# MycroftAI/mycroft-precise

Measured on AMD Instinct MI355X. Metric: MFCC+GRU windows/sec (node); max concurrent real-time 16 kHz streams, higher is better.
Workload: dtype f32

## Files before the change

include/precise_engine.h:

```cpp
#ifndef PRECISE_ENGINE_H
#define PRECISE_ENGINE_H

#include <stddef.h>
#include <stdint.h>

#ifdef __cplusplus
extern "C" {
#endif

#define PE_ABI_VERSION 8

typedef enum pe_status {
    PE_OK = 0,
    PE_ERR_INVALID = 1,
    PE_ERR_HIP = 2,
    PE_ERR_UNSUPPORTED = 3,
    PE_ERR_NOMEM = 4,
    PE_ERR_EOF = 5
} pe_status;

typedef struct pe_params {
    int32_t sample_rate;
    int32_t window_samples;
    int32_t hop_samples;
// ... 133 lines not shown
int pe_set_trigger_model(pe_engine* e, int32_t model, int32_t chunk_size_bytes, double sensitivity, int32_t trigger_level);
int pe_decode_device(pe_engine* e, const float* raw_dev, double* conf_out_dev, unsigned char* fired_out_dev, void* hip_stream);
int pe_decode(pe_engine* e, const float* raw_host, double* conf_out_host, unsigned char* fired_out_host);

typedef struct pe_info {
    int32_t n_streams, n_features, n_mfcc, units, n_layers, ring_slots, carry_capacity;
    int32_t mfcc_precision, gru_precision;
    int64_t device_bytes;
} pe_info;
int pe_get_info(const pe_engine* e, pe_info* out);

int pe_get_stream_state(pe_engine* e, int32_t* q_out, uint32_t* computed_out, uint32_t* emitted_out);

int pe_set_renumber_at(pe_engine* e, uint32_t call_number);

int pe_set_fused(pe_engine* e, int32_t enabled);

int pe_set_input_projection(pe_engine* e, int32_t enabled);

int pe_set_gru_waves(pe_engine* e, int32_t waves_per_tile);

int pe_set_gru_tiling(pe_engine* e, int32_t tiling);
int pe_get_gru_tiling(const pe_engine* e);

int pe_set_timing(pe_engine* e, int32_t enabled);
int pe_get_last_timing(pe_engine* e, float* mfcc_ms, float* gru_ms);

#define PE_TRAIN_MAX_MODELS 16
typedef struct pe_trainer pe_trainer;
int pe_trainer_create(int32_t n_features, int32_t feature_size, const pe_weights* init, int32_t device, pe_trainer** out);
int pe_trainer_create_models(int32_t n_features, int32_t feature_size, const pe_weights* init, int32_t n_models, int32_t device,
                             pe_trainer** out);
int pe_trainer_create_wide(int32_t n_features, int32_t feature_size, const pe_weights* init, int32_t n_models, int32_t device,
                           pe_trainer** out);
int pe_trainer_destroy(pe_trainer* t);
const char* pe_trainer_last_error(const pe_trainer* t);
int pe_trainer_n_models(const pe_trainer* t);
int pe_trainer_n_params(const pe_trainer* t);
int pe_trainer_n_params_model(const pe_trainer* t, int32_t m);

int pe_trainer_get_weights(pe_trainer* t, float* flat_out);
int pe_trainer_set_weights(pe_trainer* t, const float* flat);
int pe_trainer_get_accumulators(pe_trainer* t, float* flat_out);
int pe_trainer_reset_optimizer(pe_trainer* t);

int pe_trainer_loss_grad(pe_trainer* t, const float* feats_host, const float* targets_host, int32_t n, const float* masks_host,
// ... 124 lines not shown
```

mycroft_precise_amd/_lib.py:

```python
import ctypes as C
import importlib.util
import os
import weakref

import numpy as np

HERE = os.path.dirname(os.path.abspath(__file__))
LIB_PATH = os.environ.get('PE_LIB') or os.path.join(HERE, 'libprecise_engine.so')

PE_OK, PE_ERR_INVALID, PE_ERR_HIP, PE_ERR_UNSUPPORTED, PE_ERR_NOMEM, PE_ERR_EOF = range(6)
ABI_VERSION = 8


class PeParams(C.Structure):
    _fields_ = [(n, C.c_int32) for n in (
        'sample_rate', 'window_samples', 'hop_samples', 'n_fft', 'n_filt', 'n_mfcc', 'n_features',
        'use_delta', 'mfcc_precision', 'gru_precision', 'vectorizer', 'ring_precision')]


class PeGruLayer(C.Structure):
    _fields_ = [('n_in', C.c_int32), ('units', C.c_int32),
                ('kernel', C.POINTER(C.c_float)), ('recurrent_kernel', C.POINTER(C.c_float)),
                ('bias', C.POINTER(C.c_float))]

# ... 71 lines not shown
    'pe_evaluate_clips': (C.c_int, [C.c_void_p, C.c_void_p, C.c_int32, C.c_void_p, C.c_int32, C.c_int32, C.c_void_p, C.c_int64]),
    'pe_simulate_scores': (C.c_int, [C.c_void_p, C.c_void_p, C.c_int64, C.c_void_p, C.c_int32, C.c_double, C.c_double, C.c_int32,
                                     C.c_int32, C.c_void_p, C.c_int32, C.c_void_p, C.c_void_p]),
    'pe_simulate_clips': (C.c_int, [C.c_void_p, C.c_void_p, C.c_int32, C.c_void_p, C.c_int32, C.c_int32, C.c_double, C.c_double,
                                    C.c_int32, C.c_int32, C.c_void_p, C.c_int32, C.c_void_p, C.c_void_p, C.c_void_p, C.c_int64]),
    'pe_stats_scores': (C.c_int, [C.c_void_p, C.c_void_p, C.c_int32, C.c_int64, C.c_void_p, C.c_int64, C.c_void_p, C.c_int32, C.c_int32,
                                  C.c_void_p, C.c_void_p]),
    'pe_test_clips': (C.c_int, [C.c_void_p, C.c_void_p, C.c_int32, C.c_void_p, C.c_int32, C.c_int64, C.c_void_p, C.c_void_p, C.c_int32,
                                C.c_int32, C.c_void_p, C.c_void_p, C.c_void_p]),
    'pe_set_decoder': (C.c_int, [C.c_void_p, C.c_void_p, C.c_int32, C.c_int32, C.c_int32, C.c_double]),
    'pe_set_trigger': (C.c_int, [C.c_void_p, C.c_int32, C.c_double, C.c_int32]),
    'pe_set_decoder_model': (C.c_int, [C.c_void_p, C.c_int32, C.c_void_p, C.c_int32, C.c_int32, C.c_int32, C.c_double]),
    'pe_set_trigger_model': (C.c_int, [C.c_void_p, C.c_int32, C.c_int32, C.c_double, C.c_int32]),
    'pe_decode_device': (C.c_int, [C.c_void_p, C.c_void_p, C.c_void_p, C.c_void_p, C.c_void_p]),
    'pe_decode': (C.c_int, [C.c_void_p, C.c_void_p, C.c_void_p, C.c_void_p]),
    'pe_get_info': (C.c_int, [C.c_void_p, C.POINTER(PeInfo)]),
    'pe_get_stream_state': (C.c_int, [C.c_void_p, C.c_void_p, C.c_void_p, C.c_void_p]),
    'pe_set_fused': (C.c_int, [C.c_void_p, C.c_int32]),
    'pe_set_gru_waves': (C.c_int, [C.c_void_p, C.c_int32]),
    'pe_set_gru_tiling': (C.c_int, [C.c_void_p, C.c_int32]),
    'pe_get_gru_tiling': (C.c_int, [C.c_void_p]),
    'pe_set_input_projection': (C.c_int, [C.c_void_p, C.c_int32]),
    'pe_set_timing': (C.c_int, [C.c_void_p, C.c_int32]),
    'pe_get_last_timing': (C.c_int, [C.c_void_p, C.POINTER(C.c_float), C.POINTER(C.c_float)]),
    'pe_trainer_create': (C.c_int, [C.c_int32, C.c_int32, C.POINTER(PeWeights), C.c_int32, C.POINTER(C.c_void_p)]),
    'pe_trainer_destroy': (C.c_int, [C.c_void_p]),
    'pe_trainer_last_error': (C.c_char_p, [C.c_void_p]),
    'pe_trainer_n_params': (C.c_int, [C.c_void_p]),
    'pe_trainer_get_weights': (C.c_int, [C.c_void_p, C.c_void_p]),
    'pe_trainer_set_weights': (C.c_int, [C.c_void_p, C.c_void_p]),
    'pe_trainer_get_accumulators': (C.c_int, [C.c_void_p, C.c_void_p]),
    'pe_trainer_reset_optimizer': (C.c_int, [C.c_void_p]),
    'pe_trainer_loss_grad': (C.c_int, [C.c_void_p, C.c_void_p, C.c_void_p, C.c_int32, C.c_void_p, C.c_float, C.c_void_p, C.c_void_p,
                                       C.c_void_p]),
    'pe_trainer_apply': (C.c_int, [C.c_void_p, C.c_void_p, C.c_float, C.c_float, C.c_float, C.c_int32]),
    'pe_trainer_set_data': (C.c_int, [C.c_void_p, C.c_void_p, C.c_void_p, C.c_int32]),
    'pe_trainer_step': (C.c_int, [C.c_void_p, C.c_void_p, C.c_int32, C.c_float, C.c_uint64, C.c_uint64, C.c_float, C.c_float,
                                  C.c_float, C.c_float, C.c_int32, C.c_void_p]),
    'pe_trainer_evaluate': (C.c_int, [C.c_void_p, C.c_void_p, C.c_void_p, C.c_int32, C.c_float, C.c_void_p, C.c_void_p, C.c_void_p]),
    'pe_trainer_create_models': (C.c_int, [C.c_int32, C.c_int32, C.POINTER(PeWeights), C.c_int32, C.c_int32, C.POINTER(C.c_void_p)]),
    'pe_trainer_create_wide': (C.c_int, [C.c_int32, C.c_int32, C.POINTER(PeWeights), C.c_int32, C.c_int32, C.POINTER(C.c_void_p)]),
    'pe_trainer_n_models': (C.c_int, [C.c_void_p]),
    'pe_trainer_n_params_model': (C.c_int, [C.c_void_p, C.c_int32]),
    'pe_trainer_step_models': (C.c_int, [C.c_void_p, C.c_void_p, C.c_int32, C.c_uint64, C.POINTER(PeTrainHparams), C.c_void_p]),
    'pe_trainer_n_samples': (C.c_int, [C.c_void_p, C.c_int32]),
    'pe_trainer_set_validation': (C.c_int, [C.c_void_p, C.c_void_p, C.c_void_p, C.c_int32]),
# ... 549 lines not shown

    def stream_state(self):
        q = np.empty(self.n_streams, dtype=np.int32)
        kc = np.empty(self.n_streams, dtype=np.uint32)
        ke = np.empty(self.n_streams, dtype=np.uint32)
        self._check(self._lib.pe_get_stream_state(self._h, q.ctypes.data, kc.ctypes.data, ke.ctypes.data))
        return q, kc, ke

    def set_fused(self, enabled: bool):
        self._check(self._lib.pe_set_fused(self._h, int(bool(enabled))))

    def set_input_projection(self, enabled: bool):
        self._check(self._lib.pe_set_input_projection(self._h, int(bool(enabled))))

    def set_gru_waves(self, waves: int):
        self._check(self._lib.pe_set_gru_waves(self._h, int(waves)))

    def set_gru_tiling(self, tiling: int):
        self._check(self._lib.pe_set_gru_tiling(self._h, int(tiling)))

    def gru_tiling(self) -> int:
        return int(self._lib.pe_get_gru_tiling(self._h))

    def set_timing(self, enabled: bool):
        self._check(self._lib.pe_set_timing(self._h, int(bool(enabled))))

    def last_timing(self):
        a, b = C.c_float(0), C.c_float(0)
        self._check(self._lib.pe_get_last_timing(self._h, C.byref(a), C.byref(b)))
        return a.value, b.value

    def close(self):
        if getattr(self, '_h', None) and self._h.value:
            if getattr(self, '_views', 0) > 0:
                self._close_pending = True
                try:
                    self._lib.pe_wait(self._h)
                except Exception:
                    pass
                return
            for miner in list(getattr(self, '_miners', ())):
                miner.close()
            self._lib.pe_destroy(self._h)
            self._h = C.c_void_p()

    def __del__(self):
# ... 530 lines not shown
```

mycroft_precise_amd/csrc/engine.hip:

```cpp
#include "../../include/precise_engine.h"
#include "pe_common.h"
#include "gru_cw_pack.h"
#include "mfcc_general_device.h"
#include "gru_train_device.h"
#include "gru_train_wide_device.h"
#include "mine_device.h"
#include "sample_device.h"
#include "generate_device.h"
#include "augment_device.h"
#include "stats_device.h"

#include <algorithm>
#include <cmath>
#include <cstdarg>
#include <cstdio>
#include <cstdlib>
#include <cstring>
#include <string>
#include <vector>

using namespace pe;

namespace {

// ... 23 lines not shown
    double threshold = 0.5; int level = 3, rearm = -8; bool on = false;
};

}

struct pe_engine {
    pe_params prm{};
    int device = 0;
    int n_streams = 0, n_tiles = 0, n_padded = 0;
    int units = 0, n_in = 0, n_layers = 0;
    int ring_slots = 0;
    int mel_nnz = 0;
    std::string err;
    std::vector<void*> allocs;
    std::vector<size_t> alloc_bytes;
    int64_t device_bytes = 0;
    StreamRec* rec = nullptr;
    int16_t* carry = nullptr;
    const int16_t* kept = nullptr; int kept_chunk = 0;
    const int16_t* call_head = nullptr; int call_head_chunk = 0; bool call_keep = false;
    uint32_t call_no = 1;
    uint32_t renumber_at = 0x7fff0000u;
    bool fused = true;
    int gru_waves = 0;
    bool general = false;
    int row_floats = kRowFloats;
    int carry_cap = kCarryCap;
    GeneralTables gtab{};
    int gru_tiling = -1;
    int n_cus = 256;
    float* ring = nullptr;
    float* proj_ring = nullptr;
    bool proj_ok = false, proj_on = false;
    std::vector<float> proj_w_host, proj_b_host;
    int max_updates = 1;
    uint32_t* ke_hist = nullptr;
    unsigned char* table_blob = nullptr;
    pe_wave::Layout table_layout{};
    int n_models = 1;
    std::vector<NetPack> nets;
    std::vector<DecState> dec;
    bool wide = false;
    int wide_kx4[2] = {1, 1};
    int layer_units[2] = {0, 0}, layer_n_in[2] = {0, 0}, wide_units = 0;
    std::vector<double> mel_host;
    int32_t* activation = nullptr;
// ... 609 lines not shown
    WaveTables<R> t;
    t.blob = e->table_blob;
    t.L = e->table_layout;
    return t;
}

int max_frames_per_call(const pe_engine* e, long long new_samples) {
    const long long fmax = ((long long)(e->carry_cap - 1) + new_samples - frame_len_of(e->prm)) / e->prm.hop_samples + 1;
    return (int)(fmax < 1 ? 1 : fmax);
}

StreamState state_of(const pe_engine* e, uint32_t call) {
    StreamState st;
    st.rec = e->rec; st.carry = e->carry; st.n_padded = (uint32_t)e->n_padded; st.call = call;
    return st;
}

int begin_state_call(pe_engine* e, hipStream_t s, uint32_t* call) {
    if (e->call_no >= e->renumber_at) {
        PE_HIP(e, launch_renumber(state_of(e, e->call_no + 1u), e->n_padded, s));
        e->call_no = 2u;
    }
    *call = ++e->call_no;
    return PE_OK;
}

template <class R>
MfccStreamArgs<R> mfcc_args(const pe_engine* e, const int16_t* pcm_dev, int chunk, uint32_t call, const int32_t* ids = nullptr, int n_active = 0) {
    MfccStreamArgs<R> a;
    a.geo = geom(e);
    if (ids) a.geo.n_streams = n_active;
    a.pcm = pcm_dev;
    a.chunk = chunk;
    a.pcm_pairs_ok = ((chunk & 1) == 0) && ((reinterpret_cast<uintptr_t>(pcm_dev) & 3u) == 0);
    a.ids = ids;
    a.st = state_of(e, call);
    a.head = ids ? nullptr : e->call_head; a.head_chunk = e->call_head_chunk; a.keep = (!ids && e->call_keep) ? 1 : 0;
    a.ring = e->ring; a.ring_bf16 = e->prm.ring_precision;
    a.proj_ring = e->proj_on ? e->proj_ring : nullptr;
    a.n_updates = 1; a.ke_hist = nullptr; a.n_padded = e->n_padded;
    a.n_frame_rows = max_frames_per_call(e, chunk);
    a.div_hop = FastDiv::make((uint32_t)e->prm.hop_samples);
    a.div_chunk = FastDiv::make((uint32_t)chunk);
    return a;
}

// ... 195 lines not shown
int flush_kept(pe_engine* e, hipStream_t s) {
    if (!e->kept) return PE_OK;
    PE_HIP(e, launch_materialize_carry(state_of(e, e->call_no + 1u), e->kept, e->kept_chunk, e->n_streams, s));
    e->kept = nullptr; e->kept_chunk = 0;
    return PE_OK;
}

bool keep_eligible(const pe_engine* e, const int16_t* pcm_dev, int chunk) {
    return !e->general && (chunk & 1) == 0 && (reinterpret_cast<uintptr_t>(pcm_dev) & 3u) == 0 && chunk >= frame_len_of(e->prm) - 1
        && chunk >= e->carry_cap - 1;
}

bool can_fuse(const pe_engine* e, int chunk) {
    if (!(e->fused && !e->general && !e->wide && e->table_layout.mel_pad == 10 && chunk <= emit_window(e->prm) - frame_len_of(e->prm))) return false;
    if (gru_args(e).x3) return false;
    if (e->prm.gru_precision == 0 && gru_small_regs(e->units) >= 6 && gru_args(e).waves_per_tile != 4) return false;
    if (e->prm.use_delta && e->prm.gru_precision == 0) {
        const GruArgs g = gru_args(e);
        if (g.cw && (g.waves_per_tile != 4 || e->ring_slots != kCwSlots || e->prm.n_features > kCwSlots)) return false;
    }
    return true;
}

int do_update(pe_engine* e, const int16_t* pcm_dev, int chunk, float* raw_out_dev, float* feats_out_dev,
              hipStream_t s, const int32_t* ids = nullptr, int n_active = 0, bool keep = false) {
    int rc;
    const bool t = e->timing;
    const bool keep_call = keep && !ids && keep_eligible(e, pcm_dev, chunk);
    if (keep_call && e->kept) {
        const char* a0 = reinterpret_cast<const char*>(e->kept);
        const char* a1 = a0 + (size_t)e->n_streams * e->kept_chunk * sizeof(int16_t);
        const char* b0 = reinterpret_cast<const char*>(pcm_dev);
        const char* b1 = b0 + (size_t)e->n_streams * chunk * sizeof(int16_t);
        if (b0 < a1 && a0 < b1)
            return fail(e, PE_ERR_INVALID, "pe_update_device_keep: this call's chunks overlap the previous call's (%p), which still hold the "
                        "streams' leftover samples -- alternate between at least two buffers, or use pe_update_device", (const void*)e->kept);
    }
    if (!keep_call && (rc = flush_kept(e, s))) return rc;
    e->call_head = keep_call ? e->kept : nullptr; e->call_head_chunk = e->kept_chunk; e->call_keep = keep_call;
    struct Reset { pe_engine* e; ~Reset() { e->call_head = nullptr; e->call_head_chunk = 0; e->call_keep = false; } } reset{e};
    e->kept = keep_call ? pcm_dev : nullptr; e->kept_chunk = keep_call ? chunk : 0;
    uint32_t call = 0;
    if ((rc = begin_state_call(e, s, &call))) return rc;
    if (t) { PE_HIP(e, hipEventRecord(e->ev[0], s)); }
    if (raw_out_dev && can_fuse(e, chunk)) {
        GruArgs g = gru_args(e);
        g.call = call;
        g.predict_ke = 1;
        g.chunk = chunk;
        g.out = raw_out_dev;
        if (ids) { g.ids = ids; g.n_streams = n_active; }
        const ModelSet ms = model_set(e, g);
        const ModelSet* const models = e->n_models > 1 ? &ms : nullptr;
        if (e->prm.mfcc_precision == 0) PE_HIP(e, launch_fused(mfcc_args<double>(e, pcm_dev, chunk, call, ids, n_active), tables<double>(e), g, e->n_cus, s, models, e->n_models));
        else PE_HIP(e, launch_fused(mfcc_args<float>(e, pcm_dev, chunk, call, ids, n_active), tables<float>(e), g, e->n_cus, s, models, e->n_models));
        if (t) { PE_HIP(e, hipEventRecord(e->ev[1], s)); PE_HIP(e, hipEventRecord(e->ev[2], s)); e->ev_valid = true; e->ev_has_gru = false; }
    } else {
        if ((rc = launch_mfcc(e, pcm_dev, chunk, s, call, ids, n_active))) return rc;
        if (t) { PE_HIP(e, hipEventRecord(e->ev[1], s)); }
        if (raw_out_dev) {
            if ((rc = launch_gru_ring(e, raw_out_dev, s, ids, n_active))) return rc;
        }
        if (t) { PE_HIP(e, hipEventRecord(e->ev[2], s)); e->ev_valid = true; e->ev_has_gru = raw_out_dev != nullptr; }
    }
    if (feats_out_dev) {
        GatherArgs g{e->n_streams, e->prm.n_features, e->prm.n_mfcc, e->ring_slots, e->prm.ring_precision, e->ring, state_of(e, e->call_no + 1u), feats_out_dev, e->row_floats};
        PE_HIP(e, launch_gather(g, s));
    }
// ... 191 lines not shown
    if (out) *out = nullptr;
    if (n_models < 1 || n_models > kMaxModels) return fail(nullptr, PE_ERR_INVALID, "n_models must be in 1..%d, got %d", kMaxModels, n_models);
    if (!weights) return fail(nullptr, PE_ERR_INVALID, "null argument to pe_create_models");
    return create_engine(p, mel_filters, weights, n_models, n_streams, device, out);
}

int pe_get_n_models(const pe_engine* e) { return e ? e->n_models : -1; }

int pe_set_weights(pe_engine* e, const pe_weights* w, int32_t model) {
    if (!e) return PE_ERR_INVALID;
    if (!w || !w->layers || !w->dense_kernel) return fail(e, PE_ERR_INVALID, "null argument to pe_set_weights");
    if (model < 0 || model >= e->n_models) return fail(e, PE_ERR_INVALID, "model %d outside 0..%d", model, e->n_models - 1);
    if (w->n_layers != e->n_layers) return fail(e, PE_ERR_INVALID, "pe_set_weights: n_layers=%d, the engine's network has %d", w->n_layers, e->n_layers);
    for (int l = 0; l < e->n_layers; ++l) {
        const pe_gru_layer& L = w->layers[l];
        if (!L.kernel || !L.recurrent_kernel || !L.bias) return fail(e, PE_ERR_INVALID, "pe_set_weights: null weight pointer");
        if (L.units != e->layer_units[l] || L.n_in != e->layer_n_in[l])
            return fail(e, PE_ERR_INVALID, "pe_set_weights: layer %d is n_in=%d units=%d, the engine's is n_in=%d units=%d (a live engine takes the widths it was created with)",
                        l, L.n_in, L.units, e->layer_n_in[l], e->layer_units[l]);
    }
    PE_HIP(e, hipSetDevice(e->device));
    PE_DRAIN(e);
    PE_HIP(e, hipDeviceSynchronize());
    int rc = pack_model(e, e->nets[(size_t)model], w, e->wide, e->wide_units);
    if (rc) return rc;
    if (e->proj_ok && model == 0 && !e->general) {
        pack_projection_rows(e, w->layers[0]);
        rc = e->prm.mfcc_precision == 0 ? build_tables<double>(e, e->mel_host.data()) : build_tables<float>(e, e->mel_host.data());
        if (rc) return rc;
        if (e->proj_on)
            PE_HIP(e, launch_project_rows(e->ring, e->proj_ring, reinterpret_cast<const float*>(e->table_blob + e->table_layout.proj_w),
                                          reinterpret_cast<const float*>(e->table_blob + e->table_layout.proj_b), e->prm.n_mfcc,
                                          (long long)e->n_tiles * e->ring_slots * kTileStreams, nullptr));
        PE_HIP(e, hipStreamSynchronize(nullptr));
    }
    return PE_OK;
}

int pe_destroy(pe_engine* e) {
    if (!e) return PE_OK;
    (void)hipSetDevice(e->device);
    (void)drain_async(e);
    for (void* p : e->allocs) (void)hipFree(p);
    for (DeviceBuf* b : {&e->st_pcm, &e->st_out, &e->st_feats, &e->st_mask, &e->st_audio, &e->st_mfcc, &e->st_conf, &e->st_fired, &e->st_ids, &e->st_clips, &e->st_recs, &e->st_pred, &e->st_sim, &e->st_simw, &e->st_stats})
        if (b->p) (void)hipFree(b->p);
    for (auto& ev : e->ev) if (ev) (void)hipEventDestroy(ev);
// ... 1005 lines not shown
    PE_HIP(e, hipDeviceSynchronize());
    const int pending = pending_frames(e->prm);
    const long long frames = ((long long)max_updates * max_chunk_samples + e->prm.hop_samples - 1) / e->prm.hop_samples + 1;
    const int slots = next_pow2((int)(e->prm.n_features + pending + frames));
    if (slots != e->ring_slots) {
        dev_free(e, e->ring, ring_floats(e) * sizeof(float));
        e->ring = nullptr;
        dev_free(e, e->proj_ring, (size_t)e->n_tiles * e->ring_slots * kTileStreams * kProjRow * sizeof(float));
        e->proj_ring = nullptr;
        e->ring_slots = slots;
        int rc = dev_alloc(e, &e->ring, ring_floats(e));
        if (rc) return rc;
        if (e->proj_on && (rc = dev_alloc(e, &e->proj_ring, (size_t)e->n_tiles * e->ring_slots * kTileStreams * kProjRow))) return rc;
    }
    if (!e->ke_hist || max_updates > e->max_updates) {
        if (e->ke_hist) {
            dev_free(e, e->ke_hist, (size_t)e->max_updates * e->n_padded * sizeof(uint32_t));
            e->ke_hist = nullptr;
        }
        int rc = dev_alloc(e, &e->ke_hist, (size_t)max_updates * e->n_padded);
        if (rc) return rc;
    }
    e->max_updates = max_updates;
    return pe_clear(e, nullptr);
}

int pe_update_many_device(pe_engine* e, const int16_t* pcm_dev, int32_t chunk, int32_t n_updates, float* raw_out_dev, void* stream) {
    int rc = check_chunk(e, pcm_dev, chunk);
    if (rc) return rc;
    if (!raw_out_dev || n_updates < 1) return fail(e, PE_ERR_INVALID, "bad arguments to pe_update_many_device");
    if (n_updates > e->max_updates || !e->ke_hist) return fail(e, PE_ERR_INVALID, "call pe_reserve_updates(e, >= %d, >= %d) first", n_updates, chunk);
    PE_HIP(e, hipSetDevice(e->device));
    PE_DRAIN(e);
    const int flen = frame_len_of(e->prm);
    const int pending = pending_frames(e->prm);
    const long long frames = ((long long)n_updates * chunk + e->prm.hop_samples - 1) / e->prm.hop_samples + 1;
    if ((long long)n_updates * chunk >= (1ll << 30)) return fail(e, PE_ERR_INVALID, "n_updates * chunk_samples must stay below 2^30");
    if (e->prm.n_features + pending + frames > e->ring_slots) return fail(e, PE_ERR_INVALID, "reserved ring too small for %d updates of %d samples", n_updates, chunk);
    hipStream_t s = static_cast<hipStream_t>(stream);
    note_user_stream(e, stream);
    if ((rc = flush_kept(e, s))) return rc;
    uint32_t call = 0;
    if ((rc = begin_state_call(e, s, &call))) return rc;
    if (e->general) {
        if (e->prm.mfcc_precision == 0) {
            GeneralStreamArgs<double> a = general_args<double>(e, pcm_dev, chunk, call);
// ... 88 lines not shown
    PE_HIP(e, hipMemcpy(host.data(), e->rec, host.size() * sizeof(StreamRec), hipMemcpyDeviceToHost));
    const uint32_t call = e->call_no + 1u;
    for (int s = 0; s < e->n_streams; ++s) {
        const StreamRec& r0 = host[rec_at((uint32_t)e->n_padded, s, 0)];
        const StreamRec& r1 = host[rec_at((uint32_t)e->n_padded, s, 1)];
        const StreamRec& c = (call - r1.wcall) - 1u < (call - r0.wcall) - 1u ? r1 : r0;
        if (q_out) q_out[s] = c.q;
        if (computed_out) computed_out[s] = c.kc;
        if (emitted_out) emitted_out[s] = c.ke;
    }
    return PE_OK;
}

int pe_set_renumber_at(pe_engine* e, uint32_t call_number) {
    if (!e) return PE_ERR_INVALID;
    if (call_number < 8u || call_number > 0x7fff0000u) return fail(e, PE_ERR_INVALID, "renumbering threshold must be in 8..0x7fff0000");
    e->renumber_at = call_number;
    return PE_OK;
}

int pe_set_fused(pe_engine* e, int32_t enabled) {
    if (!e) return PE_ERR_INVALID;
    PE_DRAIN(e);
    e->fused = enabled != 0;
    return PE_OK;
}

int pe_set_input_projection(pe_engine* e, int32_t enabled) {
    if (!e) return PE_ERR_INVALID;
    if (enabled != 0 && enabled != 1) return fail(e, PE_ERR_INVALID, "input projection must be 0 or 1");
    if (enabled && !e->proj_ok) return fail(e, PE_ERR_UNSUPPORTED, "input-projection rows exist for the float32 network of 17..20 units without delta features only");
    if (enabled && e->n_models > 1) return fail(e, PE_ERR_UNSUPPORTED, "input-projection rows are per model: an engine of %d models has none", e->n_models);
    if ((enabled != 0) == e->proj_on) return PE_OK;
    PE_HIP(e, hipSetDevice(e->device));
    PE_DRAIN(e);
    PE_HIP(e, hipDeviceSynchronize());
    e->proj_on = enabled != 0;
    if (e->proj_on && !e->proj_ring) {
        int rc = dev_alloc(e, &e->proj_ring, (size_t)e->n_tiles * e->ring_slots * kTileStreams * kProjRow);
        if (rc) { e->proj_on = false; return rc; }
    }
    return pe_clear(e, nullptr);
}

int pe_set_gru_waves(pe_engine* e, int32_t waves) {
    if (!e) return PE_ERR_INVALID;
    if (waves != 0 && waves != 1 && waves != 4) return fail(e, PE_ERR_INVALID, "gru kernel shape must be 0 (auto), 1 or 4 (waves per tile)");
    PE_DRAIN(e);
    e->gru_waves = waves;
    return PE_OK;
}

int pe_set_gru_tiling(pe_engine* e, int32_t tiling) {
    if (!e) return PE_ERR_INVALID;
    if (tiling < -1 || tiling > 2) return fail(e, PE_ERR_INVALID, "gru tiling must be -1 (auto), 0 (classic), 1 (re-tiled) or 2 (XDL form)");
    if (e->wide && e->prm.gru_precision == 1) {
        if (tiling != 0) return fail(e, PE_ERR_UNSUPPORTED, "the bf16-operand wide network (gru_precision = 1) has one form, 0; forms 0 (f32-input MFMAs) and 2 (float32 products on the bf16 pipe) belong to the float32 wide network");
        return PE_OK;
    }
    if (e->wide) {
        if (tiling == 1) return fail(e, PE_ERR_UNSUPPORTED, "wide networks have two forms: 0 (f32-input MFMAs) and 2 (float32 products on the bf16 pipe)");
        PE_DRAIN(e);
        e->gru_tiling = tiling;
        return PE_OK;
    }
    if (tiling == 2 && !e->nets[0].x3_blob)
        return fail(e, PE_ERR_UNSUPPORTED, "the XDL form of the float32 network (tiling 2) takes <= 20 units, <= 15 inputs, float32 operands, no use_delta");
    if (tiling == 1 && e->prm.gru_precision == 1 && !e->nets[0].b20_blob)
        return fail(e, PE_ERR_UNSUPPORTED, "the five-values layout of the bf16 network (tiling 1) takes <= 20 units and <= 14 features");
    PE_DRAIN(e);
    e->gru_tiling = tiling;
    return PE_OK;
}

int pe_get_gru_tiling(const pe_engine* e) {
    if (!e) return -2;
    if (e->wide) return e->prm.gru_precision == 0 && wide_uses_x3(e) ? 2 : 0;
    if (e->prm.gru_precision != 0) return gru_args(e).b20 ? 1 : 0;
    const GruArgs a = gru_args(e);
    return a.x3 ? 2 : a.cw ? 1 : 0;
}

int pe_set_timing(pe_engine* e, int32_t enabled) {
    if (!e) return PE_ERR_INVALID;
    e->timing = enabled != 0;
    e->ev_valid = false;
    return PE_OK;
}

int pe_get_last_timing(pe_engine* e, float* mfcc_ms, float* gru_ms) {
    if (!e) return PE_ERR_INVALID;
    if (!e->ev_valid) return fail(e, PE_ERR_INVALID, "no timed update recorded (call pe_set_timing(e, 1) first)");
    PE_HIP(e, hipEventSynchronize(e->ev[2]));
    float a = 0.f, b = 0.f;
    PE_HIP(e, hipEventElapsedTime(&a, e->ev[0], e->ev[1]));
    PE_HIP(e, hipEventElapsedTime(&b, e->ev[1], e->ev[2]));
    if (mfcc_ms) *mfcc_ms = a;
    if (gru_ms) *gru_ms = e->ev_has_gru ? b : 0.f;
    return PE_OK;
}

}

static_assert(PE_TRAIN_MAX_MODELS == kTrainMaxModels, "the header's cap is the kernel table's length");

struct TrainSet {
    const float* feats = nullptr;
    const float* targets = nullptr;
    int n = 0;
// ... 1681 lines not shown
```

mycroft_precise_amd/csrc/kernels.hip:

```cpp
#include <cstdlib>
#include <type_traits>
#include "mfcc_device.h"
#include "mfcc_wave_device.h"
#include "gru_device.h"
#include "gru_cw_device.h"
#include "gru_bf16_device.h"
#include "gru_b20_device.h"
#include "gru_x3_device.h"
#include "gru_wide_device.h"
#include "gru_wide_x3_device.h"
#include "gru_wide_bf16_device.h"
#include "mfcc_general_device.h"
#include "gru_train_device.h"

namespace pe {

#ifndef PE_FRAME_WPE
#define PE_FRAME_WPE 4
#endif
template <int BYTES>
__device__ __forceinline__ void touch_kernel_arguments() {
    const int* ka = (const int*)__builtin_amdgcn_kernarg_segment_ptr();
    static_assert(BYTES <= 12 * 64, "more lines than this helper requests");
    auto line = [&](int i) -> int { return i * 64 < BYTES ? ka[i * 16] : 0; };
    const int v0 = line(0), v1 = line(1), v2 = line(2), v3 = line(3), v4 = line(4), v5 = line(5), v6 = line(6), v7 = line(7),
              v8 = line(8), v9 = line(9), v10 = line(10), v11 = line(11);
    asm volatile("" :: "s"(v0), "s"(v1), "s"(v2), "s"(v3), "s"(v4), "s"(v5), "s"(v6), "s"(v7), "s"(v8), "s"(v9), "s"(v10), "s"(v11));
}
// ... 352 lines not shown
        } else {
            const int tile = bl * 4 + wave;
            if (tile < n_tiles) gru_tile<RG, kRing, PROJ>(gm, tile, threadIdx.x & 63);
        }
    } else if (b < n_net + n_frame_blocks) {
        mfcc_frame_tasks<R, SH, true, !PROJ>(m, t, smem, (b - n_net) * kFrameWaves, n_frame_blocks * kFrameWaves, CW && MW && (frames_first & kBySimd));
    } else {
        mfcc_book_tile<R>(m, b - n_net - n_frame_blocks);
    }
}

#define PE_FUSED_PARAMS (const MfccStreamArgs<R> m, const WaveTables<R> t, const GruArgs g, const int n_gru_blocks, const int n_frame_blocks, const int n_tiles, const int frames_first)
#define PE_FUSED_MODELS_PARAMS (const MfccStreamArgs<R> m, const WaveTables<R> t, const GruArgs g, const int n_gru_blocks, const int n_models, const int n_frame_blocks, \
                                const int n_tiles, const int frames_first, const ModelSet ms)
PE_KERNEL_PAIR((template <class R, class SH, bool DELTA, bool RB>), PE_FRAME_KERNEL(256, PE_FRAME_WPE), fused_update_bf16_kernel, PE_FUSED_PARAMS,
               { fused_update_bf16_body<R, SH, DELTA, RB, false>(m, t, g, nullptr, n_gru_blocks, 1, n_frame_blocks, n_tiles, frames_first); })
PE_KERNEL_PAIR((template <class R, class SH, bool DELTA, bool RB>), PE_FRAME_KERNEL(256, PE_FRAME_WPE), fused_update_bf16_models_kernel, PE_FUSED_MODELS_PARAMS,
               { fused_update_bf16_body<R, SH, DELTA, RB, true>(m, t, g, &ms, n_gru_blocks, n_models, n_frame_blocks, n_tiles, frames_first); })
PE_KERNEL_PAIR((template <class R, class SH, int RG, bool MW, bool PROJ, bool CW = false>), PE_FRAME_KERNEL(256, PE_FRAME_WPE), fused_update_kernel, PE_FUSED_PARAMS,
               { fused_update_body<R, SH, RG, MW, PROJ, CW, false>(m, t, g, nullptr, n_gru_blocks, 1, n_frame_blocks, n_tiles, frames_first); })
PE_KERNEL_PAIR((template <class R, class SH, int RG, bool MW, bool CW>), PE_FRAME_KERNEL(256, PE_FRAME_WPE), fused_update_models_kernel, PE_FUSED_MODELS_PARAMS,
               { fused_update_body<R, SH, RG, MW, false, CW, true>(m, t, g, &ms, n_gru_blocks, n_models, n_frame_blocks, n_tiles, frames_first); })


static int frame_blocks(long long n_tasks, int n_cus, int per_cu = 4) {
    const long long need = (n_tasks + kFrameWaves - 1) / kFrameWaves;
    const long long cap = (long long)n_cus * per_cu;
    return (int)(need < cap ? (need < 1 ? 1 : need) : cap);
}

static int stream_frame_blocks(int n_streams, int n_cus, int per_cu_default = 4) {
    const long long slots = 2LL * n_streams;
    const long long cap_waves = (long long)frame_blocks(slots, n_cus, per_cu_default) * kFrameWaves;
    const long long per_wave = (slots + cap_waves - 1) / cap_waves;
    const long long waves = (slots + per_wave - 1) / per_wave;
    return (int)((waves + kFrameWaves - 1) / kFrameWaves);
}

template <class R>
static size_t frame_lds(const WaveTables<R>& t) { return wave_lds_bytes(sizeof(R), t.L, kFrameWaves); }
template <class R>
static bool blob_matches_shape(const WaveTables<R>& t) {
    return t.L.mel_pad == ShapeStock::MEL ? shape_layout_matches<R, ShapeStock>(t.L) : shape_layout_matches<R, ShapeAny>(t.L);
}

template <class R>
// ... 194 lines not shown
    if (t.L.mel_pad != ShapeStock::MEL || !blob_matches_shape(t)) return hipErrorInvalidValue;
    if (g.bf16) {
        const int tiles = (m.geo.n_streams + kTileStreams - 1) / kTileStreams;
        const int tpw = 4;
        const int gru_blocks = (tiles + tpw - 1) / tpw;
        const int ff = tiles >= 4 * n_cus ? 1 : 0;
        const int frames_first = (ff & 1) | (tpw << 8);
        const FusedLaunch f{ms, n_models, stream_frame_blocks(m.geo.n_streams, n_cus, ff ? 3 : 4), tiles, s};
        with_flag(g.use_delta, [&](auto D) { with_flag(g.ring_bf16, [&](auto RB) {
            PE_FUSED(fused_update_bf16_kernel, fused_update_bf16_models_kernel, (ShapeStock, PE_CONST(D), PE_CONST(RB)), (ShapeStock, PE_CONST(D), PE_CONST(RB)),
                     gru_blocks, frame_lds(t), frames_first); }); });
        return hipGetLastError();
    }
    hipError_t err = hipErrorInvalidValue;
    with_const<1, 2, 3, 4, 5, 6, 7, 8>(gru_small_regs(g.units), [&](auto RG) { err = launch_fused_rg<R, PE_CONST(RG)>(m, t, g, n_cus, s, ms, n_models); });
    return err;
}

hipError_t launch_fused(const MfccStreamArgs<double>& m, const WaveTables<double>& t, const GruArgs& g, int n_cus, hipStream_t s, const ModelSet* ms, int n_models) {
    return launch_fused_t<double>(m, t, g, n_cus, s, ms, n_models);
}
hipError_t launch_fused(const MfccStreamArgs<float>& m, const WaveTables<float>& t, const GruArgs& g, int n_cus, hipStream_t s, const ModelSet* ms, int n_models) {
    return launch_fused_t<float>(m, t, g, n_cus, s, ms, n_models);
}

#ifndef PE_GEN_TWO_WAVES
#define PE_GEN_TWO_WAVES 0
#endif
template <class R, int BITS, bool BLUE = false>
__global__ __launch_bounds__(64) __attribute__((amdgpu_waves_per_eu(BITS >= 10 ? 2 : 4))) void mfcc_general_stream_kernel(const GeneralStreamArgs<R> a) {
    extern __shared__ __attribute__((aligned(16))) unsigned char smem[];
    const int s = PE_GEN_TWO_WAVES ? blockIdx.x >> 1 : blockIdx.x;
    if (s < a.geo.n_streams) general_stream<R, BITS, BLUE>(a, reinterpret_cast<R*>(smem), s, PE_GEN_TWO_WAVES ? blockIdx.x & 1 : 0, threadIdx.x, PE_GEN_TWO_WAVES ? 2 : 1);
}
template <class R, int BITS, bool BLUE = false>
__global__ __launch_bounds__(64) __attribute__((amdgpu_waves_per_eu(BITS >= 10 ? 2 : 4))) PE_NO_PK_F32 void mfcc_general_stream_kernel_nopk(const GeneralStreamArgs<R> a) {
    extern __shared__ __attribute__((aligned(16))) unsigned char smem[];
    const int s = PE_GEN_TWO_WAVES ? blockIdx.x >> 1 : blockIdx.x;
    if (s < a.geo.n_streams) general_stream<R, BITS, BLUE>(a, reinterpret_cast<R*>(smem), s, PE_GEN_TWO_WAVES ? blockIdx.x & 1 : 0, threadIdx.x, PE_GEN_TWO_WAVES ? 2 : 1);
}
template <class R, int BITS, bool BLUE = false>
__global__ __launch_bounds__(64) __attribute__((amdgpu_waves_per_eu(BITS >= 10 ? 2 : 4))) void mfcc_general_offline_kernel(const GeneralOfflineArgs<R> a) {
    extern __shared__ __attribute__((aligned(16))) unsigned char smem[];
    general_offline<R, BITS, BLUE>(a, reinterpret_cast<R*>(smem), blockIdx.x, gridDim.x, threadIdx.x);
}
template <class R, int BITS, bool BLUE = false>
// ... 389 lines not shown
```

mycroft_precise_amd/csrc/pe_common.h:

```cpp
#pragma once
#include <hip/hip_runtime.h>
#include <stdint.h>
#include "mfcc_wave_tables.h"

namespace pe {

constexpr int kTileStreams = 16;
constexpr int kRowFloats = 16;
constexpr int kCarryCap = 512;
constexpr int kNfft = 512;
constexpr int kBins = kNfft / 2 + 1;
constexpr int kMaxFilt = 64;
constexpr int kCwSlots = 32;

template <class R> struct cplx { R x, y; };

constexpr int kMaxFrameRows = 4096;
constexpr int kFrameWaves = 4;

template <class R>
struct WaveTables {
    const void* blob;
    pe_wave::Layout L;
};
// ... 340 lines not shown
struct DecodeArgs {
    int n_streams;
    const float* raw;
    const double* cd;
    int cd_len, min_out, out_range;
    double center;
    double* conf_out;
    int32_t* activation;
    unsigned char* fired_out;
    double threshold;
    int trigger_level, rearm;
};
hipError_t launch_decode(const DecodeArgs& a, hipStream_t s);
struct DecodeSet { DecodeArgs m[kMaxModels]; };
hipError_t launch_decode_models(const DecodeSet& d, int n_models, int n_streams, hipStream_t s);
hipError_t launch_clear_activation(const uint8_t* mask, int32_t* activation, int n_streams, int n_padded, int n_rows, hipStream_t s);

constexpr int kProjRow = pe_wave::kProjRow;
hipError_t launch_mfcc_f64(const MfccStreamArgs<double>& a, const WaveTables<double>& t, int n_cus, hipStream_t s);
hipError_t launch_mfcc_f32(const MfccStreamArgs<float>& a, const WaveTables<float>& t, int n_cus, hipStream_t s);
hipError_t launch_gru_many(const GruArgs& a, int n_updates, int n_padded, hipStream_t s, const ModelSet* ms = nullptr, int n_models = 1);
hipError_t launch_fused(const MfccStreamArgs<double>& m, const WaveTables<double>& t, const GruArgs& g, int n_cus, hipStream_t s, const ModelSet* ms = nullptr, int n_models = 1);
hipError_t launch_fused(const MfccStreamArgs<float>& m, const WaveTables<float>& t, const GruArgs& g, int n_cus, hipStream_t s, const ModelSet* ms = nullptr, int n_models = 1);
hipError_t launch_mfcc_offline_f64(const MfccOfflineArgs<double>& a, const WaveTables<double>& t, int n_cus, hipStream_t s);
hipError_t launch_mfcc_offline_f32(const MfccOfflineArgs<float>& a, const WaveTables<float>& t, int n_cus, hipStream_t s);
hipError_t launch_mfcc_clips_f64(const MfccClipArgs<double>& a, const WaveTables<double>& t, int n_cus, hipStream_t s);
hipError_t launch_mfcc_clips_f32(const MfccClipArgs<float>& a, const WaveTables<float>& t, int n_cus, hipStream_t s);
hipError_t launch_mfcc_recs_f64(const MfccRecArgs<double>& a, const WaveTables<double>& t, int n_cus, hipStream_t s);
hipError_t launch_mfcc_recs_f32(const MfccRecArgs<float>& a, const WaveTables<float>& t, int n_cus, hipStream_t s);
hipError_t launch_simulate(const SimArgs& a, int n_models, int n_cus, hipStream_t s);
hipError_t launch_gru_small(const GruArgs& a, int input_mode, hipStream_t s, const ModelSet* ms = nullptr, int n_models = 1, long long out_stride = 0);
int gru_small_regs(int units);
int gru_wide_waves(int units);
int gru_small_tiles(int units);
hipError_t launch_gru_wide(const WideArgs& a, int input_mode, hipStream_t s);
hipError_t launch_gru_wide_x3(const WideArgs& a, int input_mode, hipStream_t s);
hipError_t launch_gru_wide_bf16(const WideArgs& a, int input_mode, hipStream_t s);
hipError_t launch_gather(const GatherArgs& a, hipStream_t s);
hipError_t launch_scatter(const GatherArgs& a, hipStream_t s);
hipError_t launch_renumber(const StreamState& st, int n_padded, hipStream_t s);
hipError_t launch_materialize_carry(const StreamState& st, const int16_t* head, int head_chunk, int n_streams, hipStream_t s);
hipError_t launch_clear(const ClearArgs& a, hipStream_t s);
hipError_t launch_project_rows(const float* ring, float* proj, const float* w, const float* b, int n_mfcc, long long n_rows, hipStream_t s);

}
```

Baseline: 271.7 million.

## Carry per-offset GRU hidden-state chains across calls instead of recomputing windows

Adds a chain-carry path. For each stream and each window start offset it keeps a partial GRU hidden state in device memory, so each update only advances every chain by the one or two new frames. Without it, the GRU re-runs over the whole feature window from a zero state on every call. The change cuts the serial recurrence depth per call, and spreads the chains across four waves inside the fused MFCC+GRU kernel. In exchange it adds per-call loads and stores of the chain states and a rebuild kernel. It also needs epoch bookkeeping to invalidate the chains whenever configuration or state changes, and switches on automatically after a streak of eligible calls.

```diff
diff --git a/include/precise_engine.h b/include/precise_engine.h
--- a/include/precise_engine.h
+++ b/include/precise_engine.h
@@ -179,6 +179,9 @@
 
 int pe_set_gru_tiling(pe_engine* e, int32_t tiling);
 int pe_get_gru_tiling(const pe_engine* e);
+
+int pe_set_chain_carry(pe_engine* e, int32_t mode);
+int pe_get_chain_carry(const pe_engine* e, int32_t* mode, int32_t* active);
 
 int pe_set_timing(pe_engine* e, int32_t enabled);
 int pe_get_last_timing(pe_engine* e, float* mfcc_ms, float* gru_ms);
diff --git a/mycroft_precise_amd/_lib.py b/mycroft_precise_amd/_lib.py
--- a/mycroft_precise_amd/_lib.py
+++ b/mycroft_precise_amd/_lib.py
@@ -117,6 +117,8 @@
     'pe_get_gru_tiling': (C.c_int, [C.c_void_p]),
     'pe_set_input_projection': (C.c_int, [C.c_void_p, C.c_int32]),
     'pe_set_timing': (C.c_int, [C.c_void_p, C.c_int32]),
+    'pe_set_chain_carry': (C.c_int, [C.c_void_p, C.c_int32]),
+    'pe_get_chain_carry': (C.c_int, [C.c_void_p, C.POINTER(C.c_int32), C.POINTER(C.c_int32)]),
     'pe_get_last_timing': (C.c_int, [C.c_void_p, C.POINTER(C.c_float), C.POINTER(C.c_float)]),
     'pe_trainer_create': (C.c_int, [C.c_int32, C.c_int32, C.POINTER(PeWeights), C.c_int32, C.POINTER(C.c_void_p)]),
     'pe_trainer_destroy': (C.c_int, [C.c_void_p]),
@@ -712,6 +714,14 @@
     def gru_tiling(self) -> int:
         return int(self._lib.pe_get_gru_tiling(self._h))
 
+    def set_chain_carry(self, mode: int):
+        self._check(self._lib.pe_set_chain_carry(self._h, int(mode)))
+
+    def chain_carry(self):
+        m, a = C.c_int32(0), C.c_int32(0)
+        self._check(self._lib.pe_get_chain_carry(self._h, C.byref(m), C.byref(a)))
+        return m.value, bool(a.value)
+
     def set_timing(self, enabled: bool):
         self._check(self._lib.pe_set_timing(self._h, int(bool(enabled))))
 
diff --git a/mycroft_precise_amd/csrc/engine.hip b/mycroft_precise_amd/csrc/engine.hip
--- a/mycroft_precise_amd/csrc/engine.hip
+++ b/mycroft_precise_amd/csrc/engine.hip
@@ -69,6 +69,12 @@
     uint32_t call_no = 1;
     uint32_t renumber_at = 0x7fff0000u;
     bool fused = true;
+    int chain_mode = 1;
+    float* chains = nullptr;
+    uint32_t* chain_ke = nullptr;
+    uint64_t chain_epoch = 1, chains_built_epoch = 0;
+    int chain_streak = 0;
+    uint64_t chain_seen_epoch = 0;
     int gru_waves = 0;
     bool general = false;
     int row_floats = kRowFloats;
@@ -724,6 +730,7 @@
         e->call_no = 2u;
     }
     *call = ++e->call_no;
+    ++e->chain_epoch;
     return PE_OK;
 }
 
@@ -965,6 +972,18 @@
     return true;
 }
 
+constexpr int kChainEnterAfter = 128;
+
+bool chain_eligible(const pe_engine* e, int chunk) {
+    if (e->chain_mode == 0 || e->n_models != 1 || e->prm.use_delta || e->prm.ring_precision != 0 || e->timing) return false;
+    if (e->gru_tiling >= 0 || e->gru_waves != 0 || !e->fused || e->max_updates > 1) return false;
+    if (e->ring_slots != kCwSlots || e->prm.n_features > kCwSlots - 3) return false;
+    if ((chunk + e->prm.hop_samples - 1) / e->prm.hop_samples > 2) return false;
+    if (!can_fuse(e, chunk)) return false;
+    const GruArgs g = gru_args(e);
+    return g.cw && g.waves_per_tile == 4 && !g.proj_ring && !g.bf16 && !g.x3;
+}
+
 int do_update(pe_engine* e, const int16_t* pcm_dev, int chunk, float* raw_out_dev, float* feats_out_dev,
               hipStream_t s, const int32_t* ids = nullptr, int n_active = 0, bool keep = false) {
     int rc;
@@ -983,10 +1002,32 @@
     e->call_head = keep_call ? e->kept : nullptr; e->call_head_chunk = e->kept_chunk; e->call_keep = keep_call;
     struct Reset { pe_engine* e; ~Reset() { e->call_head = nullptr; e->call_head_chunk = 0; e->call_keep = false; } } reset{e};
     e->kept = keep_call ? pcm_dev : nullptr; e->kept_chunk = keep_call ? chunk : 0;
+    const bool chain_call = raw_out_dev && !feats_out_dev && chain_eligible(e, chunk);
+    const bool chains_current = chain_call && e->chains && e->chains_built_epoch == e->chain_epoch;
+    if (!chain_call || e->chain_epoch != e->chain_seen_epoch) e->chain_streak = 0;
+    if (chain_call) ++e->chain_streak;
+    const bool chains_enter = chain_call && !chains_current && (e->chain_mode == 2 || e->chain_streak > kChainEnterAfter);
     uint32_t call = 0;
     if ((rc = begin_state_call(e, s, &call))) return rc;
+    e->chain_seen_epoch = e->chain_epoch;
     if (t) { PE_HIP(e, hipEventRecord(e->ev[0], s)); }
-    if (raw_out_dev && can_fuse(e, chunk)) {
+    if (chains_current || chains_enter) {
+        if (!e->chains) {
+            if ((rc = dev_alloc(e, &e->chain_ke, (size_t)e->n_padded))) return rc;
+            if ((rc = dev_alloc(e, &e->chains, (size_t)e->n_tiles * kCwSlots * 5 * 64))) return rc;
+        }
+        const ChainArgs ch{e->chains, e->chain_ke};
+        GruArgs g = gru_args(e);
+        g.call = call;
+        if (chains_enter) PE_HIP(e, launch_chains_rebuild(g, ch, e->n_padded, s));
+        g.predict_ke = 1;
+        g.chunk = chunk;
+        g.out = raw_out_dev;
+        if (ids) { g.ids = ids; g.n_streams = n_active; }
+        if (e->prm.mfcc_precision == 0) PE_HIP(e, launch_fused_chains(mfcc_args<double>(e, pcm_dev, chunk, call, ids, n_active), tables<double>(e), g, ch, e->n_cus, s));
+        else PE_HIP(e, launch_fused_chains(mfcc_args<float>(e, pcm_dev, chunk, call, ids, n_active), tables<float>(e), g, ch, e->n_cus, s));
+        e->chains_built_epoch = e->chain_epoch;
+    } else if (raw_out_dev && can_fuse(e, chunk)) {
         GruArgs g = gru_args(e);
         g.call = call;
         g.predict_ke = 1;
@@ -1224,6 +1265,7 @@
     PE_HIP(e, hipSetDevice(e->device));
     PE_DRAIN(e);
     PE_HIP(e, hipDeviceSynchronize());
+    ++e->chain_epoch;
     int rc = pack_model(e, e->nets[(size_t)model], w, e->wide, e->wide_units);
     if (rc) return rc;
     if (e->proj_ok && model == 0 && !e->general) {
@@ -2275,6 +2317,7 @@
         if (rc) return rc;
     }
     e->max_updates = max_updates;
+    ++e->chain_epoch;
     return pe_clear(e, nullptr);
 }
 
@@ -2409,6 +2452,7 @@
 int pe_set_fused(pe_engine* e, int32_t enabled) {
     if (!e) return PE_ERR_INVALID;
     PE_DRAIN(e);
+    ++e->chain_epoch;
     e->fused = enabled != 0;
     return PE_OK;
 }
@@ -2423,6 +2467,7 @@
     PE_DRAIN(e);
     PE_HIP(e, hipDeviceSynchronize());
     e->proj_on = enabled != 0;
+    ++e->chain_epoch;
     if (e->proj_on && !e->proj_ring) {
         int rc = dev_alloc(e, &e->proj_ring, (size_t)e->n_tiles * e->ring_slots * kTileStreams * kProjRow);
         if (rc) { e->proj_on = false; return rc; }
@@ -2434,6 +2479,7 @@
     if (!e) return PE_ERR_INVALID;
     if (waves != 0 && waves != 1 && waves != 4) return fail(e, PE_ERR_INVALID, "gru kernel shape must be 0 (auto), 1 or 4 (waves per tile)");
     PE_DRAIN(e);
+    ++e->chain_epoch;
     e->gru_waves = waves;
     return PE_OK;
 }
@@ -2456,6 +2502,7 @@
     if (tiling == 1 && e->prm.gru_precision == 1 && !e->nets[0].b20_blob)
         return fail(e, PE_ERR_UNSUPPORTED, "the five-values layout of the bf16 network (tiling 1) takes <= 20 units and <= 14 features");
     PE_DRAIN(e);
+    ++e->chain_epoch;
     e->gru_tiling = tiling;
     return PE_OK;
 }
@@ -2472,6 +2519,24 @@
     if (!e) return PE_ERR_INVALID;
     e->timing = enabled != 0;
     e->ev_valid = false;
+    ++e->chain_epoch;
+    return PE_OK;
+}
+
+int pe_set_chain_carry(pe_engine* e, int32_t mode) {
+    if (!e) return PE_ERR_INVALID;
+    if (mode < 0 || mode > 2) return fail(e, PE_ERR_INVALID, "chain carry must be 0 (off), 1 (automatic) or 2 (eager)");
+    PE_DRAIN(e);
+    ++e->chain_epoch;
+    e->chain_streak = 0;
+    e->chain_mode = mode;
+    return PE_OK;
+}
+
+int pe_get_chain_carry(const pe_engine* e, int32_t* mode, int32_t* active) {
+    if (!e) return PE_ERR_INVALID;
+    if (mode) *mode = e->chain_mode;
+    if (active) *active = (e->chain_mode != 0 && e->chains && e->chains_built_epoch == e->chain_epoch) ? 1 : 0;
     return PE_OK;
 }
 
diff --git a/mycroft_precise_amd/csrc/gru_chain_device.h b/mycroft_precise_amd/csrc/gru_chain_device.h
--- /dev/null
+++ b/mycroft_precise_amd/csrc/gru_chain_device.h
@@ -0,0 +1,156 @@
+#pragma once
+#include "gru_cw_device.h"
+
+namespace pe {
+
+constexpr int kChainMaxRows = 2;
+
+__device__ __forceinline__ size_t chain_cell(const long long sid, const uint32_t slot, const int g) {
+    return (((size_t)(sid >> 4) * kCwSlots + slot) * 5) * 64 + (size_t)(g * 16) + (size_t)(sid & 15);
+}
+__device__ __forceinline__ void chain_load(const float* chains, const size_t cell, float (&h)[5]) {
+#pragma unroll
+    for (int rho = 0; rho < 5; ++rho) h[rho] = chains[cell + (size_t)rho * 64];
+}
+__device__ __forceinline__ void chain_store(float* chains, const size_t cell, const float (&h)[5], const bool on) {
+    if (!on) return;
+#pragma unroll
+    for (int rho = 0; rho < 5; ++rho) chains[cell + (size_t)rho * 64] = h[rho];
+}
+
+struct ChainNet {
+    CwStep<false> S;
+    float wx[4][4];
+    f32x4 bias[4];
+    __device__ __forceinline__ void load(const float* cw, const int lane) {
+        S.load(cw, lane);
+#pragma unroll
+        for (int tl = 0; tl < 4; ++tl)
+#pragma unroll
+            for (int kk = 0; kk < 4; ++kk) {
+                wx[tl][kk] = cw[CwPack::WX + (tl * 4 + kk) * 64 + lane];
+                bias[tl][kk] = cw[CwPack::BIAS + (tl * 4 + kk) * 64 + lane];
+            }
+    }
+    __device__ __forceinline__ void project(const f32x4& x, f32x4 (&p)[4]) const {
+        p[kTZ] = cw_xproj(wx[kTZ], bias[kTZ], x); p[kTX] = cw_xproj(wx[kTX], bias[kTX], x);
+        p[kTC] = cw_xproj(wx[kTC], bias[kTC], x); p[kTV] = cw_xproj(wx[kTV], bias[kTV], x);
+    }
+    __device__ __forceinline__ void step_if(float (&h)[5], const f32x4 (&p)[4], const bool on) const {
+        float hn[5];
+#pragma unroll
+        for (int rho = 0; rho < 5; ++rho) hn[rho] = h[rho];
+        S.step(hn, p[kTZ], p[kTX], p[kTC], p[kTV]);
+#pragma unroll
+        for (int rho = 0; rho < 5; ++rho) h[rho] = on ? hn[rho] : h[rho];
+    }
+};
+
+template <int NW>
+__device__ __forceinline__ void gru_tile_chains(const GruArgs& a, const ChainArgs& ch, const int tile, const int wave, const int lane) {
+    const int g = lane >> 4, j = lane & 15;
+    const long long stream = (long long)tile * kTileStreams + j;
+    const bool valid = stream < a.n_streams;
+    const int T = a.n_features;
+    const long long sid = gru_stream_of(a, stream, valid);
+    const KeRequest ke_req = gru_ke_request(a, sid);
+    const uint32_t stamp = ch.chain_ke[sid];
+    ChainNet N;
+    N.load(a.cw, lane);
+    float wd[5];
+#pragma unroll
+    for (int rho = 0; rho < 5; ++rho) wd[rho] = a.wd[rho * 64 + lane];
+    const uint32_t ke_pre = rec_pick(ke_req.p, rec_side(ke_req.p, a.call)).ke;
+    const uint32_t ke_post = gru_ke_resolve(a, ke_req);
+    const uint32_t k = ke_post - ke_pre;
+    const int kmax = __any(k >= 2u) ? 2 : __any(k >= 1u) ? 1 : 0;
+    const int head_wave = T % NW;
+    constexpr bool kAhead = NW > 4;
+    const uint32_t smask = (uint32_t)(kCwSlots - 1);
+    const float* xbase = a.ring + gru_ring_cell(a, sid) * kRowFloats + 4 * g;
+    f32x4 p0[4], p1[4];
+    if (kmax >= 1) N.project(*reinterpret_cast<const f32x4*>(xbase + (size_t)(ke_pre & smask) * kTileStreams * kRowFloats), p0);
+    if (kmax >= 2) N.project(*reinterpret_cast<const f32x4*>(xbase + (size_t)((ke_pre + 1u) & smask) * kTileStreams * kRowFloats), p1);
+    auto advance = [&](float (&h)[5], const uint32_t A) {
+        if (kmax >= 1) N.step_if(h, p0, 0u < k && k <= A);
+        if (kmax >= 2) N.step_if(h, p1, 1u < k && k <= A + 1u);
+    };
+    const bool moved = valid && k > 0u;
+    float hw[5];
+#pragma unroll
+    for (int rho = 0; rho < 5; ++rho) hw[rho] = 0.f;
+    if (kmax == 0) {
+        if (wave == head_wave) chain_load(ch.chains, chain_cell(sid, (ke_post - (uint32_t)T) & smask, g), hw);
+    } else {
+        auto cell_of = [&](const int age) -> size_t { return chain_cell(sid, (ke_post - (uint32_t)(age <= T ? age : T)) & smask, g); };
+        const int first = wave ? wave : NW;
+        float n0[5], n1[5];
+        if (kAhead) {
+            chain_load(ch.chains, cell_of(first), n0);
+            chain_load(ch.chains, cell_of(first + NW), n1);
+        }
+        for (int a0 = first; a0 <= T; a0 += 2 * NW) {
+            const uint32_t A0 = (uint32_t)a0, A1 = A0 + (uint32_t)NW;
+            const bool two = a0 + NW <= T;
+            const size_t c0 = cell_of(a0), c1 = cell_of(a0 + NW);
+            float h0[5], h1[5];
+            if (!kAhead) {
+                chain_load(ch.chains, c0, n0);
+                chain_load(ch.chains, c1, n1);
+            }
+#pragma unroll
+            for (int rho = 0; rho < 5; ++rho) {
+                h0[rho] = A0 <= k ? 0.f : n0[rho];
+                h1[rho] = A1 <= k ? 0.f : n1[rho];
+            }
+            if (kAhead && a0 + 2 * NW <= T) {
+                chain_load(ch.chains, cell_of(a0 + 2 * NW), n0);
+                chain_load(ch.chains, cell_of(a0 + 3 * NW), n1);
+            }
+            advance(h0, A0);
+            if (two) advance(h1, A1);
+            chain_store(ch.chains, c0, h0, moved);
+            if (two) chain_store(ch.chains, c1, h1, moved);
+            if (a0 == T) {
+#pragma unroll
+                for (int rho = 0; rho < 5; ++rho) hw[rho] = h0[rho];
+            }
+            if (two && a0 + NW == T) {
+#pragma unroll
+                for (int rho = 0; rho < 5; ++rho) hw[rho] = h1[rho];
+            }
+        }
+    }
+    if (wave == head_wave) {
+        if (stamp != ke_pre || k > (uint32_t)kChainMaxRows) hw[0] = __builtin_nanf("");
+        cw_head(a, hw, wd, stream, valid, g);
+        if (valid && g == 0) ch.chain_ke[sid] = ke_post;
+    }
+}
+
+__device__ __forceinline__ void gru_tile_chains_rebuild(const GruArgs& a, const ChainArgs& ch, const int tile, const int wave, const int lane) {
+    const int g = lane >> 4, j = lane & 15;
+    const long long sid = (long long)tile * kTileStreams + j;
+    const int T = a.n_features;
+    const KeRequest ke_req = gru_ke_request(a, sid);
+    ChainNet N;
+    N.load(a.cw, lane);
+    const uint32_t ke = gru_ke_resolve(a, ke_req);
+    const uint32_t smask = (uint32_t)(kCwSlots - 1);
+    const float* xbase = a.ring + gru_ring_cell(a, sid) * kRowFloats + 4 * g;
+    for (int a0 = wave ? wave : 4; a0 <= T; a0 += 4) {
+        float h[5];
+#pragma unroll
+        for (int rho = 0; rho < 5; ++rho) h[rho] = 0.f;
+        const uint32_t start = ke - (uint32_t)a0;
+        for (int i = 0; i < a0; ++i) {
+            f32x4 p[4];
+            N.project(*reinterpret_cast<const f32x4*>(xbase + (size_t)((start + (uint32_t)i) & smask) * kTileStreams * kRowFloats), p);
+            N.S.step(h, p[kTZ], p[kTX], p[kTC], p[kTV]);
+        }
+        chain_store(ch.chains, chain_cell(sid, start & smask, g), h, true);
+    }
+    if (wave == 0 && g == 0) ch.chain_ke[sid] = ke;
+}
+
+}
diff --git a/mycroft_precise_amd/csrc/kernels.hip b/mycroft_precise_amd/csrc/kernels.hip
--- a/mycroft_precise_amd/csrc/kernels.hip
+++ b/mycroft_precise_amd/csrc/kernels.hip
@@ -4,6 +4,7 @@
 #include "mfcc_wave_device.h"
 #include "gru_device.h"
 #include "gru_cw_device.h"
+#include "gru_chain_device.h"
 #include "gru_bf16_device.h"
 #include "gru_b20_device.h"
 #include "gru_x3_device.h"
@@ -402,6 +403,32 @@
 PE_KERNEL_PAIR((template <class R, class SH, int RG, bool MW, bool CW>), PE_FRAME_KERNEL(256, PE_FRAME_WPE), fused_update_models_kernel, PE_FUSED_MODELS_PARAMS,
                { fused_update_body<R, SH, RG, MW, false, CW, true>(m, t, g, &ms, n_gru_blocks, n_models, n_frame_blocks, n_tiles, frames_first); })
 
+template <class R, class SH, int NW>
+__device__ __forceinline__ void fused_update_chains_body(const MfccStreamArgs<R>& m, const WaveTables<R>& t, const GruArgs& g, const ChainArgs& ch,
+                                                         const int n_gru_blocks, const int n_frame_blocks, const int frames_first) {
+    extern __shared__ __attribute__((aligned(16))) unsigned char smem[];
+    touch_kernel_arguments<kFusedArgBytes<R, false> + (int)sizeof(ChainArgs)>();
+    const int b = role_block(blockIdx.x, n_gru_blocks, n_frame_blocks, frames_first & kFramesFirst);
+    if (b < n_gru_blocks) {
+        constexpr int per_tile = NW / 4;
+        const int wave = __builtin_amdgcn_readfirstlane(threadIdx.x >> 6) + 4 * (b % per_tile);
+        gru_tile_chains<NW>(g, ch, b / per_tile, wave, threadIdx.x & 63);
+    } else if (b < n_gru_blocks + n_frame_blocks) {
+        __builtin_amdgcn_s_setprio(3);
+        mfcc_frame_tasks<R, SH, true, true>(m, t, smem, (b - n_gru_blocks) * kFrameWaves, n_frame_blocks * kFrameWaves, false);
+    } else {
+        mfcc_book_tile<R>(m, b - n_gru_blocks - n_frame_blocks);
+    }
+}
+PE_KERNEL_PAIR((template <class R, class SH, int NW>), PE_FRAME_KERNEL(256, PE_FRAME_WPE), fused_update_chains_kernel,
+               (const MfccStreamArgs<R> m, const WaveTables<R> t, const GruArgs g, const int n_gru_blocks, const int n_frame_blocks, const int n_tiles,
+                const int frames_first, const ChainArgs ch),
+               { (void)n_tiles; fused_update_chains_body<R, SH, NW>(m, t, g, ch, n_gru_blocks, n_frame_blocks, frames_first); })
+__global__ __launch_bounds__(256) void gru_chains_rebuild_kernel(const GruArgs a, const ChainArgs ch) {
+    const int wave = __builtin_amdgcn_readfirstlane(threadIdx.x >> 6);
+    gru_tile_chains_rebuild(a, ch, blockIdx.x, wave, threadIdx.x & 63);
+}
+
 
 static int frame_blocks(long long n_tasks, int n_cus, int per_cu = 4) {
     const long long need = (n_tasks + kFrameWaves - 1) / kFrameWaves;
@@ -642,6 +669,31 @@
 }
 hipError_t launch_fused(const MfccStreamArgs<float>& m, const WaveTables<float>& t, const GruArgs& g, int n_cus, hipStream_t s, const ModelSet* ms, int n_models) {
     return launch_fused_t<float>(m, t, g, n_cus, s, ms, n_models);
+}
+
+template <class R>
+static hipError_t launch_fused_chains_t(const MfccStreamArgs<R>& m, const WaveTables<R>& t, const GruArgs& g, const ChainArgs& ch, int n_cus, hipStream_t s) {
+    if (t.L.mel_pad != ShapeStock::MEL || !blob_matches_shape(t)) return hipErrorInvalidValue;
+    if (!g.cw || g.waves_per_tile != 4 || !cw_four_waves_ok(g) || !g.predict_ke || !ch.chains || !ch.chain_ke) return hipErrorInvalidValue;
+    const int tiles = (m.geo.n_streams + kTileStreams - 1) / kTileStreams;
+    if (tiles == 0) return hipSuccess;
+    const int fb = stream_frame_blocks(m.geo.n_streams, n_cus, tiles <= n_cus ? 2 : 4);
+    const bool sparse = g.ids && 2u * (uint32_t)tiles * kTileStreams <= g.n_padded;
+    if (sparse) PE_LAUNCH_R(R, fused_update_chains_kernel, (ShapeStock, 8), dim3(2 * tiles + fb + tiles), dim3(256), frame_lds(t), s, m, t, g, 2 * tiles, fb, tiles, 0, ch);
+    else PE_LAUNCH_R(R, fused_update_chains_kernel, (ShapeStock, 4), dim3(tiles + fb + tiles), dim3(256), frame_lds(t), s, m, t, g, tiles, fb, tiles, 0, ch);
+    return hipGetLastError();
+}
+hipError_t launch_fused_chains(const MfccStreamArgs<double>& m, const WaveTables<double>& t, const GruArgs& g, const ChainArgs& ch, int n_cus, hipStream_t s) {
+    return launch_fused_chains_t<double>(m, t, g, ch, n_cus, s);
+}
+hipError_t launch_fused_chains(const MfccStreamArgs<float>& m, const WaveTables<float>& t, const GruArgs& g, const ChainArgs& ch, int n_cus, hipStream_t s) {
+    return launch_fused_chains_t<float>(m, t, g, ch, n_cus, s);
+}
+hipError_t launch_chains_rebuild(const GruArgs& a, const ChainArgs& ch, int n_padded, hipStream_t s) {
+    if (!a.cw || !cw_four_waves_ok(a) || a.ids || a.predict_ke || !ch.chains || !ch.chain_ke) return hipErrorInvalidValue;
+    if (n_padded == 0) return hipSuccess;
+    hipLaunchKernelGGL(gru_chains_rebuild_kernel, dim3(n_padded / kTileStreams), dim3(256), 0, s, a, ch);
+    return hipGetLastError();
 }
 
 #ifndef PE_GEN_TWO_WAVES
diff --git a/mycroft_precise_amd/csrc/pe_common.h b/mycroft_precise_amd/csrc/pe_common.h
--- a/mycroft_precise_amd/csrc/pe_common.h
+++ b/mycroft_precise_amd/csrc/pe_common.h
@@ -386,6 +386,13 @@
 hipError_t launch_gru_many(const GruArgs& a, int n_updates, int n_padded, hipStream_t s, const ModelSet* ms = nullptr, int n_models = 1);
 hipError_t launch_fused(const MfccStreamArgs<double>& m, const WaveTables<double>& t, const GruArgs& g, int n_cus, hipStream_t s, const ModelSet* ms = nullptr, int n_models = 1);
 hipError_t launch_fused(const MfccStreamArgs<float>& m, const WaveTables<float>& t, const GruArgs& g, int n_cus, hipStream_t s, const ModelSet* ms = nullptr, int n_models = 1);
+struct ChainArgs {
+    float* chains;
+    uint32_t* chain_ke;
+};
+hipError_t launch_fused_chains(const MfccStreamArgs<double>& m, const WaveTables<double>& t, const GruArgs& g, const ChainArgs& ch, int n_cus, hipStream_t s);
+hipError_t launch_fused_chains(const MfccStreamArgs<float>& m, const WaveTables<float>& t, const GruArgs& g, const ChainArgs& ch, int n_cus, hipStream_t s);
+hipError_t launch_chains_rebuild(const GruArgs& a, const ChainArgs& ch, int n_padded, hipStream_t s);
 hipError_t launch_mfcc_offline_f64(const MfccOfflineArgs<double>& a, const WaveTables<double>& t, int n_cus, hipStream_t s);
 hipError_t launch_mfcc_offline_f32(const MfccOfflineArgs<float>& a, const WaveTables<float>& t, int n_cus, hipStream_t s);
 hipError_t launch_mfcc_clips_f64(const MfccClipArgs<double>& a, const WaveTables<double>& t, int n_cus, hipStream_t s);
```

New measurement: 288.8 million (median of 6 runs). 6.3% higher.
